# gregbugaj/marie-icr

Measured on AMD Instinct MI355X. Metric: pages/sec (2550x3300, ~40 lines/page), higher is better.
Workload: dtype f16; 1 GPU; BASELINE configs[2]: full detect->crop->recognize, 64 synthetic 2550x3300x3 u8 pages per GPU per step resident in HBM; DiT-base Mask R-CNN detector (resize to 1035x800, 1 pass, 8 pages per forward) + TrOCR-base recognizer on the generator's 40 ground-truth line boxes per page (fixed work), beam 3, 15+1 decoder steps; seeded random weights; f16 operands with fp32 accumulation is the 16-bit mode of ; crops_per_page=40

## Files before the change

### include/marie_hip.h

```cpp
#ifndef MARIE_HIP_H
#define MARIE_HIP_H

#include <stddef.h>
#include <stdint.h>

#ifdef __cplusplus
extern "C" {
#endif

#define MHIP_OK 0
#define MHIP_EINVAL (-22)
#define MHIP_ENOMEM (-12)
#define MHIP_EHIP (-5)
#define MHIP_ESTATE (-1)

#define MHIP_PREC_F16 0
#define MHIP_PREC_F32 1

typedef struct mhip_ctx mhip_ctx;
typedef struct mhip_crnn mhip_crnn;

int mhip_init(int device_id, mhip_ctx** out);
int mhip_destroy(mhip_ctx* ctx);
const char* mhip_last_error(mhip_ctx* ctx);
int mhip_set_stream(mhip_ctx* ctx, void* hip_stream);
int mhip_synchronize(mhip_ctx* ctx);
int mhip_device_info(mhip_ctx* ctx, char* arch, size_t arch_len, int* cu_count, size_t* hbm_bytes);
int mhip_memcpy_dev(mhip_ctx* ctx, void* dst_dev, const void* src_dev, size_t bytes);

typedef struct mhip_gate mhip_gate;
int mhip_gate_create(mhip_ctx* ctx, mhip_gate** out);
int mhip_gate_destroy(mhip_gate* g);
int mhip_gate_signal(mhip_gate* g, mhip_ctx* ctx);
long long mhip_gate_count(mhip_gate* g);
int mhip_gate_open(mhip_gate* g, int open);
int mhip_gate_wait(mhip_gate* g, mhip_ctx* ctx, long long seq, int timeout_ms);

int mhip_profile_enable(mhip_ctx* ctx, int enable);
int mhip_profile_reset(mhip_ctx* ctx);
int mhip_profile_read(mhip_ctx* ctx, int kernel_id, double* total_ms, int64_t* launches);
int mhip_profile_flops(mhip_ctx* ctx, int kernel_id, double* flops);
int mhip_kernel_count(void);
const char* mhip_kernel_name(int kernel_id);

typedef struct mhip_conv_desc {
  int32_t B, H, W, Cin;
  int32_t KH, KW, pad;
  int32_t N;
  int32_t pool, relu, out_f32;
  int32_t dil;
  int32_t Cin1;
  int32_t ldc;
  int32_t pad_cols_writable;
} mhip_conv_desc;
int mhip_conv2d_nhwc(mhip_ctx* ctx, int precision, const mhip_conv_desc* d, const void* in_dev,
                     const void* in2_dev, const void* w_dev, const float* scale_dev, const float* bias_dev,
                     void* out_dev);
typedef struct mhip_conv_ex_desc {
  int32_t B, H, W, Cin;
  int32_t KH, KW, pad;
  int32_t N;
  int32_t pool, relu, out_f32;
  int32_t dil;
  int32_t Cin1;
  int32_t ldc;
  int32_t pad_cols_writable;
  int32_t sy;
  int32_t pad_x;
  int32_t row_period, row_stride, row_offset;
  const void* res_dev;
} mhip_conv_ex_desc;
int mhip_conv2d_nhwc_ex(mhip_ctx* ctx, int precision, const mhip_conv_ex_desc* d, const void* in_dev,
                        const void* in2_dev, const void* w_dev, const float* scale_dev, const float* bias_dev,
                        void* out_dev);

typedef struct mhip_crop_desc {
  uint64_t src_offset;
  int32_t h, w, row_stride, channels;
} mhip_crop_desc;
// ... 359 lines not shown
```

### marie_icr_amd/_lib.py

```python
from __future__ import annotations

import ctypes as C
import os
import weakref

import numpy as np

_HERE = os.path.dirname(os.path.abspath(__file__))
LIB_PATH = os.environ.get("MARIE_HIP_LIB") or os.path.join(_HERE, "libmarie_hip.so")

PREC_F16 = 0
PREC_F32 = 1

_vp, _i, _sz = C.c_void_p, C.c_int, C.c_size_t
_SIGNATURES = (
    ("mhip_init", _i, [_i, C.POINTER(_vp)]),
    ("mhip_destroy", _i, [_vp]),
    ("mhip_last_error", C.c_char_p, [_vp]),
    ("mhip_set_stream", _i, [_vp, _vp]),
    ("mhip_synchronize", _i, [_vp]),
    ("mhip_device_info", _i, [_vp, C.c_char_p, _sz, C.POINTER(_i), C.POINTER(_sz)]),
    ("mhip_memcpy_dev", _i, [_vp, _vp, _vp, _sz]),
    ("mhip_gate_create", _i, [_vp, C.POINTER(_vp)]),
    ("mhip_gate_destroy", _i, [_vp]),
    ("mhip_gate_signal", _i, [_vp, _vp]),
    ("mhip_gate_count", C.c_longlong, [_vp]),
    ("mhip_gate_open", _i, [_vp, _i]),
    ("mhip_gate_wait", _i, [_vp, _vp, C.c_longlong, _i]),
    ("mhip_profile_enable", _i, [_vp, _i]),
    ("mhip_profile_reset", _i, [_vp]),
    ("mhip_profile_read", _i, [_vp, _i, C.POINTER(C.c_double), C.POINTER(C.c_int64)]),
    ("mhip_profile_flops", _i, [_vp, _i, C.POINTER(C.c_double)]),
    ("mhip_kernel_count", _i, []),
    ("mhip_kernel_name", C.c_char_p, [_i]),
    ("mhip_conv2d_nhwc", _i, [_vp, _i, _vp, _vp, _vp, _vp, _vp, _vp, _vp]),
    ("mhip_conv2d_nhwc_ex", _i, [_vp, _i, _vp, _vp, _vp, _vp, _vp, _vp, _vp]),
    ("mhip_icr_create", _i, [_vp, _i, _i, C.POINTER(_vp)]),
    ("mhip_icr_destroy", _i, [_vp]),
    ("mhip_icr_set_tensor", _i, [_vp, C.c_char_p, _vp, C.POINTER(C.c_int64), _i]),
    ("mhip_icr_finalize", _i, [_vp]),
    ("mhip_icr_alloc_arena", _i, [_vp]),
    ("mhip_icr_arena", _i, [_vp, C.POINTER(_vp), C.POINTER(_sz)]),
    ("mhip_icr_steps", _i, []),
    ("mhip_icr_forward", _i, [_vp, _vp, _i, _vp, _vp, _vp, _vp]),
    ("mhip_icr_forward_host", _i, [_vp, _vp, _i, _vp, _vp, _vp, _vp]),
    ("mhip_craft_create", _i, [_vp, _i, C.POINTER(_vp)]),
    ("mhip_craft_destroy", _i, [_vp]),
    ("mhip_craft_set_tensor", _i, [_vp, C.c_char_p, _vp, C.POINTER(C.c_int64), _i]),
    ("mhip_craft_finalize", _i, [_vp]),
    ("mhip_craft_alloc_arena", _i, [_vp]),
    ("mhip_craft_arena", _i, [_vp, C.POINTER(_vp), C.POINTER(_sz)]),
    ("mhip_craft_geometry", _i, [_i, _i, _i, C.c_double, C.POINTER(C.c_double), C.POINTER(_i), C.POINTER(_i),
                                 C.POINTER(_i), C.POINTER(_i)]),
    ("mhip_craft_workspace_bytes", _sz, [_vp, _i, _i, _i, C.c_double]),
    ("mhip_craft_kernel_flops", C.c_double, [_vp, _i, _i, _i, _i, C.c_double]),
    ("mhip_craft_forward", _i, [_vp, _vp, _i, _i, _i, C.c_double, _vp]),
    ("mhip_craft_detect", _i, [_vp, _vp, _i, _i, _i, C.c_double, C.c_float, C.c_float, C.c_float, _vp, _i,
                               C.POINTER(_i), _vp, C.POINTER(C.c_double)]),
    ("mhip_craft_detect_host", _i, [_vp, _vp, _i, _i, _i, C.c_double, C.c_float, C.c_float, C.c_float, _vp, _i,
                                    C.POINTER(_i), _vp, C.POINTER(C.c_double)]),
    ("mhip_craft_boxes_host", _i, [_vp, _vp, _i, _i, C.c_float, C.c_float, C.c_float, _vp, _i, C.POINTER(_i), _vp, _vp,
                                   _vp, _i, C.POINTER(_i)]),
    ("mhip_crop_batch", _i, [_vp, _vp, _vp, _i, _i, _vp]),
    ("mhip_pil_resize_rgb_host", _i, [_vp, _vp, _i, _i, _vp, _i, _i, _i]),
    ("mhip_pil_resize_fragments_host", _i, [_vp, _vp, _sz, _vp, _i, _i, _i, _i, _vp]),
    ("mhip_vit_create", _i, [_vp, _i, _vp, C.POINTER(_vp)]),
    ("mhip_vit_destroy", _i, [_vp]),
    ("mhip_vit_set_tensor", _i, [_vp, C.c_char_p, _vp, C.POINTER(C.c_int64), _i]),
    ("mhip_vit_finalize", _i, [_vp]),
    ("mhip_vit_alloc_arena", _i, [_vp]),
    ("mhip_vit_arena", _i, [_vp, C.POINTER(_vp), C.POINTER(_sz)]),
    ("mhip_vit_forward_host", _i, [_vp, _vp, _i, _i, _i, _i, _i, _i, _vp, _vp, _vp, _vp, _vp]),
    ("mhip_dit_default_config", _i, [_i, _vp]),
# ... 139 lines not shown


class VitConfig(C.Structure):
    _fields_ = [("dim", C.c_int), ("depth", C.c_int), ("heads", C.c_int), ("patch", C.c_int), ("pos_h", C.c_int),
                ("pos_w", C.c_int), ("layer_scale", C.c_int), ("qkv_bias", C.c_int), ("final_norm", C.c_int),
                ("fpn", C.c_int), ("taps", C.c_int * 4), ("ln_eps", C.c_float)]


class DitConfig(C.Structure):
    _fields_ = [("model", C.c_int), ("min_size_test", C.c_int), ("max_size_test", C.c_int),
                ("detections_per_image", C.c_int), ("anchor_sizes", C.c_float * 5), ("aspect_ratios", C.c_float * 3),
                ("rpn_nms_thresh", C.c_float), ("score_thresh", C.c_float), ("nms_thresh", C.c_float),
                ("num_classes", C.c_int)]


class RegisterDesc(C.Structure):
    _fields_ = [("crop_x", C.c_int), ("crop_y", C.c_int), ("crop_w", C.c_int), ("crop_h", C.c_int), ("out_w", C.c_int),
                ("out_h", C.c_int), ("left", C.c_int), ("top", C.c_int), ("canvas_w", C.c_int), ("canvas_h", C.c_int),
                ("n_markers", C.c_int), ("marker_x", C.c_int * 4), ("marker_y", C.c_int * 4), ("marker_radius", C.c_int),
                ("marker_color", C.c_int * 3), ("final_w", C.c_int), ("final_h", C.c_int)]


class TrocrConfig(C.Structure):
    _fields_ = [("enc_dim", C.c_int), ("enc_depth", C.c_int), ("enc_heads", C.c_int), ("dec_dim", C.c_int),
                ("dec_layers", C.c_int), ("dec_heads", C.c_int), ("dec_ffn", C.c_int), ("vocab", C.c_int),
                ("max_positions", C.c_int), ("beam", C.c_int), ("max_len_b", C.c_int), ("min_len", C.c_int),
                ("pad", C.c_int), ("eos", C.c_int), ("embed_scale", C.c_float), ("img_size", C.c_int)]


class LayoutLMv3Config(C.Structure):
    _fields_ = [("hidden", C.c_int), ("layers", C.c_int), ("heads", C.c_int), ("ffn", C.c_int), ("vocab", C.c_int),
                ("type_vocab", C.c_int), ("max_position_embeddings", C.c_int), ("max_2d_position_embeddings", C.c_int),
                ("coordinate_size", C.c_int), ("shape_size", C.c_int), ("input_size", C.c_int), ("patch", C.c_int),
                ("rel_pos_bins", C.c_int), ("max_rel_pos", C.c_int), ("rel_2d_pos_bins", C.c_int),
                ("max_rel_2d_pos", C.c_int), ("layer_norm_eps", C.c_float), ("pad_id", C.c_int), ("num_labels", C.c_int),
                ("max_text", C.c_int)]


class ClipVisConfig(C.Structure):
    _fields_ = [("dim", C.c_int), ("depth", C.c_int), ("heads", C.c_int), ("patch", C.c_int), ("image_size", C.c_int),
                ("ffn", C.c_int), ("proj_dim", C.c_int), ("ln_eps", C.c_float)]


class VqFilters(C.Structure):
    _fields_ = [("n", C.c_int32), ("taps", (C.c_float * 16) * 6), ("dil", (C.c_int32 * 2) * 6), ("weight", C.c_double * 6)]


class CropDesc(C.Structure):
    _fields_ = [("src_offset", C.c_uint64), ("h", C.c_int32), ("w", C.c_int32), ("row_stride", C.c_int32),
                ("channels", C.c_int32)]


POOL_NONE, POOL_2x2, POOL_2x1 = 0, 1, 2

_lib = None


class MarieHipError(RuntimeError):
    pass


def load():
    global _lib
    if _lib is not None:
        return _lib
    import importlib.util
    import sys

    if "torch" not in sys.modules and importlib.util.find_spec("torch") is not None:
        import torch
    if not os.path.exists(LIB_PATH):
        raise MarieHipError(
            f"{LIB_PATH} is missing — the HIP extension is not built; there is no CPU fallback "
            "(run __graft_entry__.build() or `make -C marie_icr_amd/csrc`)")
    lib = C.CDLL(LIB_PATH)
    for name, res, args in _SIGNATURES:
        fn = getattr(lib, name)
        fn.restype = res
        fn.argtypes = args
    _lib = lib
    return lib


def check(ctx_handle, rc: int, what: str):
    if rc != 0:
        msg = load().mhip_last_error(ctx_handle)
        raise MarieHipError(f"{what} failed ({rc}): {msg.decode() if msg else ''}")


class Context:

    def __init__(self, device_id: int = 0):
        lib = load()
        h = C.c_void_p()
        rc = lib.mhip_init(int(device_id), C.byref(h))
        if rc != 0 or not h.value:
            raise MarieHipError(f"mhip_init(device={device_id}) failed ({rc}): no usable HIP device")
        self.h = h
        self.lib = lib
        self.device_id = int(device_id)
        self._children = weakref.WeakSet()

    def adopt(self, child):
        self._children.add(child)

    def set_stream(self, stream_handle: int | None):
        check(self.h, self.lib.mhip_set_stream(self.h, C.c_void_p(stream_handle or 0)), "mhip_set_stream")

    def synchronize(self):
        check(self.h, self.lib.mhip_synchronize(self.h), "mhip_synchronize")

    def device_info(self):
        arch = C.create_string_buffer(64)
        cu = C.c_int()
        hbm = C.c_size_t()
        check(self.h, self.lib.mhip_device_info(self.h, arch, 64, C.byref(cu), C.byref(hbm)), "mhip_device_info")
        return {"arch": arch.value.decode(), "cu_count": cu.value, "hbm_bytes": hbm.value}

    def memcpy_dev(self, dst_ptr: int, src_ptr: int, nbytes: int):
        check(self.h, self.lib.mhip_memcpy_dev(self.h, C.c_void_p(dst_ptr), C.c_void_p(src_ptr), int(nbytes)),
              "mhip_memcpy_dev")

    def conv2d_nhwc(self, precision: int, desc: "ConvDesc", in_ptr: int, w_ptr: int, scale_ptr: int, bias_ptr: int,
                    out_ptr: int, in2_ptr: int = 0):
        check(self.h, self.lib.mhip_conv2d_nhwc(self.h, int(precision), C.byref(desc), C.c_void_p(in_ptr),
                                                C.c_void_p(in2_ptr or 0), C.c_void_p(w_ptr), C.c_void_p(scale_ptr or 0),
                                                C.c_void_p(bias_ptr or 0), C.c_void_p(out_ptr)),
              "mhip_conv2d_nhwc")

    def conv2d_nhwc_ex(self, precision: int, desc: "ConvExDesc", in_ptr: int, w_ptr: int, scale_ptr: int, bias_ptr: int,
                       out_ptr: int, in2_ptr: int = 0):
        check(self.h, self.lib.mhip_conv2d_nhwc_ex(self.h, int(precision), C.byref(desc), C.c_void_p(in_ptr),
                                                   C.c_void_p(in2_ptr or 0), C.c_void_p(w_ptr), C.c_void_p(scale_ptr or 0),
                                                   C.c_void_p(bias_ptr or 0), C.c_void_p(out_ptr)),
              "mhip_conv2d_nhwc_ex")

    def gemm_ln_fold(self, precision: int, desc: "GemmFoldDesc"):
        check(self.h, self.lib.mhip_gemm_ln_fold(self.h, int(precision), C.byref(desc)), "mhip_gemm_ln_fold")

    def ln_finalize(self, stats_ptr: int, chunks: int, ld: int, rstd_ptr: int, mur_ptr: int, rows: int, D: int, eps: float):
        check(self.h, self.lib.mhip_ln_finalize(self.h, C.c_void_p(stats_ptr), int(chunks), int(ld), C.c_void_p(rstd_ptr),
                                                C.c_void_p(mur_ptr), int(rows), int(D), float(eps)), "mhip_ln_finalize")

    def token_init_split(self, hi_ptr: int, lo_ptr: int, cls_row_ptr: int, cls_stats_ptr: int, stats_ptr: int, stats_ld: int,
                         B: int, npad: int, n_tok: int, D: int):
        check(self.h, self.lib.mhip_token_init_split(self.h, C.c_void_p(hi_ptr), C.c_void_p(lo_ptr), C.c_void_p(cls_row_ptr),
                                                     C.c_void_p(cls_stats_ptr), C.c_void_p(stats_ptr), int(stats_ld), int(B),
                                                     int(npad), int(n_tok), int(D)), "mhip_token_init_split")

    def profile_enable(self, on: bool):
        check(self.h, self.lib.mhip_profile_enable(self.h, 1 if on else 0), "mhip_profile_enable")

    def profile_reset(self):
        check(self.h, self.lib.mhip_profile_reset(self.h), "mhip_profile_reset")

    def profile_read(self):
        out = {}
        for k in range(self.lib.mhip_kernel_count()):
            ms = C.c_double()
            n = C.c_int64()
            check(self.h, self.lib.mhip_profile_read(self.h, k, C.byref(ms), C.byref(n)), "mhip_profile_read")
            fl = C.c_double()
            check(self.h, self.lib.mhip_profile_flops(self.h, k, C.byref(fl)), "mhip_profile_flops")
            out[self.lib.mhip_kernel_name(k).decode()] = {"id": k, "total_ms": ms.value, "launches": n.value,
# ... 107 lines not shown
```

### marie_icr_amd/csrc/common.h

```cpp
#pragma once
#include <hip/hip_runtime.h>
#include <stdint.h>
#include <stdio.h>
#include <string.h>

#include <mutex>
#include <string>
#include <vector>

#include "../../include/marie_hip.h"

enum MhipKernelId {
  MHIP_K_CONV_FIRST = 0,
  MHIP_K_CONV_IGEMM = 1,
  MHIP_K_LSTM_REC = 2,
  MHIP_K_CTC_DECODE = 3,
  MHIP_K_IMAGE_OPS = 4,
  MHIP_K_CCL = 5,
  MHIP_K_CROP_BATCH = 6,
  MHIP_K_ATTN = 7,
  MHIP_K_ATTN_FLASH = 8,
  MHIP_K_VIT_OPS = 9,
  MHIP_K_DET_OPS = 10,
  MHIP_K_DEC_OPS = 11,
  MHIP_K_IGEMM_T64 = 12,
  MHIP_K_IGEMM_T128 = 13,
  MHIP_K_IGEMM_T256 = 14,
  MHIP_K_IGEMM_S128 = 15,
  MHIP_K_IGEMM_PATCH = 16,
  MHIP_K_CROSS_ATTN = 17,
  MHIP_K_ATTN_BIAS = 18,
  MHIP_K_VQ_ASSIGN = 19,
  MHIP_K_VQ_KMEANS = 20,
  MHIP_K_VQ_HEATMAP = 21,
  MHIP_K_VQ_PEAKS = 22,
  MHIP_K_CLIP_COSINE = 23,
  MHIP_K_CLIPVIS_PATCHIFY = 24,
  MHIP_K_CLIPVIS_EMBED = 25,
  MHIP_K_QUICK_GELU = 26,
  MHIP_K_CLIPVIS_HEAD = 27,
  MHIP_K_PAIR_COSINE = 28,
  MHIP_K_COUNT = 29
};

constexpr int MHIP_ZERO_BYTES = 65536;

struct ProfSlot {
  double total_ms = 0.0;
  int64_t launches = 0;
  double flops = 0.0;
  int parent = -1;
  std::vector<std::pair<hipEvent_t, hipEvent_t>> pending;
};

struct mhip_ctx {
  int device = 0;
  hipStream_t stream = nullptr;
  std::string err;
  void* ws = nullptr;
  size_t ws_bytes = 0;
  void* zeros = nullptr;
  bool profiling = false;
  ProfSlot prof[MHIP_K_COUNT];
  std::vector<hipEvent_t> event_pool;
  struct PinnedRing {
    static constexpr int N = 4;
    void* buf[N] = {nullptr, nullptr, nullptr, nullptr};
    size_t cap[N] = {0, 0, 0, 0};
    hipEvent_t ev[N] = {nullptr, nullptr, nullptr, nullptr};
    int next = 0;
  } stage;
};
int mhip_stage_h2d(mhip_ctx* ctx, void* dst_dev, const void* src_host, size_t bytes);

int mhip_fail(mhip_ctx* ctx, int code, const char* fmt, ...);
inline void mhip_quiesce(const mhip_ctx* ctx) {
  if (ctx) (void)hipSetDevice(ctx->device);
  (void)hipDeviceSynchronize();
}
int mhip_ensure_workspace(mhip_ctx* ctx, size_t bytes);

struct Carver {
  char* base;
  size_t align;
  size_t off = 0;
  explicit Carver(void* b, size_t a = 256) : base((char*)b), align(a) {}
  template <typename P = char>
  P* take(size_t bytes) {
    const size_t at = off;
    off = (off + bytes + align - 1) / align * align;
    return base ? (P*)(base + at) : nullptr;
  }
  Carver sub(size_t a) const { return Carver(base ? base + off : nullptr, a); }
};

template <typename F>
size_t mhip_layout_bytes(F&& layout, size_t align = 256) {
  Carver c(nullptr, align);
  layout(c);
  return c.off;
}
template <typename F>
int mhip_carve_workspace(mhip_ctx* ctx, F&& layout, size_t align = 256) {
  const size_t need = mhip_layout_bytes(layout, align);
  int rc = mhip_ensure_workspace(ctx, need);
  if (rc) return rc;
  Carver ws(ctx->ws, align);
  layout(ws);
  if (ws.off != need) return mhip_fail(ctx, MHIP_ESTATE, "workspace layout carved %zu bytes, sized %zu", ws.off, need);
  return MHIP_OK;
}
extern "C" int mhip_gate_signal(mhip_gate* g, mhip_ctx* ctx);
void mhip_prof_begin(mhip_ctx* ctx, int kid, hipEvent_t* e0);
void mhip_prof_end(mhip_ctx* ctx, int kid, hipEvent_t e0);

// ... 379 lines not shown
```

### marie_icr_amd/csrc/context.hip

```cpp
#include <stdarg.h>

#include <algorithm>

#include "common.h"

int mhip_fail(mhip_ctx* ctx, int code, const char* fmt, ...) {
  char buf[512];
  va_list ap;
  va_start(ap, fmt);
  vsnprintf(buf, sizeof(buf), fmt, ap);
  va_end(ap);
  if (ctx) ctx->err = buf;
  return code;
}

static const char* kKernelNames[MHIP_K_COUNT] = {"conv_first", "conv_igemm", "lstm_rec",   "ctc_decode",
                                                 "image_ops",  "ccl",        "crop_batch", "attn",
                                                 "attn_flash", "vit_ops",    "det_ops",    "dec_ops",
                                                 "conv_igemm<64>", "conv_igemm<128>", "conv_igemm<256>", "conv_igemm<1128>",
                                                 "conv3x3_patch", "cross_attn", "attn_bias",
                                                 "vq_assign", "vq_kmeans", "vq_heatmap", "vq_peaks", "clip_cosine",
                                                 "clipvis_patchify", "clipvis_embed", "quick_gelu", "clipvis_head", "pair_cosine"};

extern "C" int mhip_kernel_count(void) { return MHIP_K_COUNT; }
extern "C" const char* mhip_kernel_name(int k) { return (k >= 0 && k < MHIP_K_COUNT) ? kKernelNames[k] : ""; }

extern "C" int mhip_init(int device_id, mhip_ctx** out) {
  if (!out) return MHIP_EINVAL;
  *out = nullptr;
  int ndev = 0;
  if (hipGetDeviceCount(&ndev) != hipSuccess || ndev <= 0) return MHIP_EHIP;
  if (device_id < 0 || device_id >= ndev) return MHIP_EINVAL;
  if (hipSetDevice(device_id) != hipSuccess) return MHIP_EHIP;
  mhip_ctx* ctx = new mhip_ctx();
  ctx->device = device_id;
  for (int k = MHIP_K_IGEMM_T64; k <= MHIP_K_IGEMM_PATCH; ++k) ctx->prof[k].parent = MHIP_K_CONV_IGEMM;
  if (hipMalloc(&ctx->zeros, MHIP_ZERO_BYTES) != hipSuccess || hipMemset(ctx->zeros, 0, MHIP_ZERO_BYTES) != hipSuccess) {
    delete ctx;
    return MHIP_ENOMEM;
  }
  *out = ctx;
  return MHIP_OK;
}

extern "C" int mhip_destroy(mhip_ctx* ctx) {
  if (!ctx) return MHIP_OK;
  (void)hipSetDevice(ctx->device);
  mhip_quiesce(ctx);
  for (auto& s : ctx->prof)
    for (auto& p : s.pending) {
      (void)hipEventDestroy(p.first);
      (void)hipEventDestroy(p.second);
    }
  for (auto e : ctx->event_pool) (void)hipEventDestroy(e);
  for (int i = 0; i < mhip_ctx::PinnedRing::N; ++i) {
    if (ctx->stage.ev[i]) (void)hipEventDestroy(ctx->stage.ev[i]);
    if (ctx->stage.buf[i]) (void)hipHostFree(ctx->stage.buf[i]);
  }
  if (ctx->ws) (void)hipFree(ctx->ws);
  if (ctx->zeros) (void)hipFree(ctx->zeros);
  delete ctx;
  return MHIP_OK;
}

int mhip_stage_h2d(mhip_ctx* ctx, void* dst_dev, const void* src_host, size_t bytes) {
  if (!bytes) return MHIP_OK;
  mhip_ctx::PinnedRing& r = ctx->stage;
  const int i = r.next;
  r.next = (i + 1) % mhip_ctx::PinnedRing::N;
  if (r.ev[i]) MHIP_HIP(ctx, hipEventSynchronize(r.ev[i]));
  else MHIP_HIP(ctx, hipEventCreateWithFlags(&r.ev[i], hipEventDisableTiming));
  if (bytes > r.cap[i]) {
    if (r.buf[i]) (void)hipHostFree(r.buf[i]);
    r.buf[i] = nullptr; r.cap[i] = 0;
    const size_t cap = std::max<size_t>(bytes, 64 * 1024);
    MHIP_HIP(ctx, hipHostMalloc(&r.buf[i], cap, hipHostMallocDefault));
    r.cap[i] = cap;
  }
  memcpy(r.buf[i], src_host, bytes);
  MHIP_HIP(ctx, hipMemcpyAsync(dst_dev, r.buf[i], bytes, hipMemcpyHostToDevice, ctx->stream));
  MHIP_HIP(ctx, hipEventRecord(r.ev[i], ctx->stream));
  return MHIP_OK;
}

extern "C" const char* mhip_last_error(mhip_ctx* ctx) { return ctx ? ctx->err.c_str() : "null ctx"; }

extern "C" int mhip_set_stream(mhip_ctx* ctx, void* s) {
  if (!ctx) return MHIP_EINVAL;
  ctx->stream = (hipStream_t)s;
  return MHIP_OK;
}

extern "C" int mhip_synchronize(mhip_ctx* ctx) {
  if (!ctx) return MHIP_EINVAL;
  MHIP_HIP(ctx, hipStreamSynchronize(ctx->stream));
  return MHIP_OK;
}

extern "C" int mhip_device_info(mhip_ctx* ctx, char* arch, size_t arch_len, int* cu_count, size_t* hbm_bytes) {
  if (!ctx) return MHIP_EINVAL;
  hipDeviceProp_t p;
  MHIP_HIP(ctx, hipGetDeviceProperties(&p, ctx->device));
  if (arch && arch_len) {
    strncpy(arch, p.gcnArchName, arch_len - 1);
    arch[arch_len - 1] = 0;
  }
  if (cu_count) *cu_count = p.multiProcessorCount;
  if (hbm_bytes) *hbm_bytes = p.totalGlobalMem;
  return MHIP_OK;
}

extern "C" int mhip_memcpy_dev(mhip_ctx* ctx, void* dst, const void* src, size_t bytes) {
  if (!ctx || (bytes && (!dst || !src))) return MHIP_EINVAL;
  MHIP_HIP(ctx, hipMemcpyAsync(dst, src, bytes, hipMemcpyDeviceToDevice, ctx->stream));
  return MHIP_OK;
}

int mhip_ensure_workspace(mhip_ctx* ctx, size_t bytes) {
  if (bytes <= ctx->ws_bytes) return MHIP_OK;
  MHIP_HIP(ctx, hipStreamSynchronize(ctx->stream));
  if (ctx->ws) MHIP_HIP(ctx, hipFree(ctx->ws));
  ctx->ws = nullptr;
  ctx->ws_bytes = 0;
  size_t want = bytes + bytes / 8;
  if (hipMalloc(&ctx->ws, want) != hipSuccess) {
    (void)hipGetLastError();
    return mhip_fail(ctx, MHIP_ENOMEM, "workspace allocation of %zu bytes failed", want);
  }
  ctx->ws_bytes = want;
  return MHIP_OK;
}

static hipEvent_t get_event(mhip_ctx* ctx) {
  if (!ctx->event_pool.empty()) {
    hipEvent_t e = ctx->event_pool.back();
    ctx->event_pool.pop_back();
    return e;
  }
  hipEvent_t e = nullptr;
  (void)hipEventCreate(&e);
  return e;
}
// ... 58 lines not shown
```

### marie_icr_amd/csrc/conv_igemm.hip

```cpp
#include <stdlib.h>

#include <type_traits>

#include "igemm_common.h"

using namespace igemm;

namespace {

template <int BN_>
struct Cfg {
  static constexpr bool SMALL = BN_ / 1000 == 1;
  static constexpr int BN = BN_ % 1000;
  static constexpr int BM = SMALL ? 128 : ((BN == 64) ? 512 : 256);
  static constexpr int WN = BN / 64;
  static constexpr int WM = 8 / WN;
  static constexpr int MT = BM / WM / 16;
  static constexpr int NSTAGE = SMALL ? 4 : ((BN == 128) ? 3 : 2);
  static constexpr int A_BYTES = BM * ROWB;
  static constexpr int B_BYTES = BN * ROWB;
  static constexpr int STAGE_BYTES = A_BYTES + B_BYTES;
  static constexpr int RPI = 64 * 16 / ROWB;
  static constexpr int ACHUNKS = BM * (ROWB / 16) / NTHREADS;
  static constexpr int WCHUNKS = BN * (ROWB / 16) / NTHREADS;
  static constexpr int GL = ACHUNKS + WCHUNKS;
  static constexpr int EPW = BN < 128 ? BN : 128;
  static constexpr int EPI_BYTES = BM * (EPW * 4 + 16);
  static constexpr int RING_BYTES = NSTAGE * STAGE_BYTES;
  static constexpr int LDS_BYTES = RING_BYTES > EPI_BYTES ? RING_BYTES : EPI_BYTES;
};

__device__ __forceinline__ float gelu_erf(float t) {
  const float x = t * 0.70710678118654752f, ax = fabsf(x);
  const float u = __builtin_amdgcn_rcpf(__builtin_fmaf(0.3275911f, ax, 1.f));
  float poly = __builtin_fmaf(1.061405429f, u, -1.453152027f);
  poly = __builtin_fmaf(poly, u, 1.421413741f);
  poly = __builtin_fmaf(poly, u, -0.284496736f);
  poly = __builtin_fmaf(poly, u, 0.254829592f);
  poly = poly * u;
  const float e = __builtin_fmaf(-poly, __builtin_amdgcn_exp2f((-1.4426950408889634f * ax) * ax), 1.f);
  const float h = 0.5f * t;
  return __builtin_fmaf(h, copysignf(e, x), h);
}

template <int CTRL>
__device__ __forceinline__ float dpp_f(float v) {
  return __builtin_bit_cast(float, __builtin_amdgcn_update_dpp(0, __builtin_bit_cast(int, v), CTRL, 0xf, 0xf, true));
}
__device__ __forceinline__ float sum8(float v) {
  v += dpp_f<0xB1>(v);
  v += dpp_f<0x4E>(v);
  v += dpp_f<0x141>(v);
  return v;
}


__device__ __forceinline__ void staged8(const char* src, float (&f)[8]) {
  const float4v a0 = *(const float4v*)src, a1 = *(const float4v*)(src + 16);
  f[0] = a0[0]; f[1] = a0[1]; f[2] = a0[2]; f[3] = a0[3]; f[4] = a1[0]; f[5] = a1[1]; f[6] = a1[2]; f[7] = a1[3];
}


template <bool SMALL, typename V, typename P>
__device__ __forceinline__ void tile_store(const V& v, P dst) {
  if (SMALL) *dst = v;
  else __builtin_nontemporal_store(v, dst);
}

template <int POOL>
__device__ __forceinline__ void decode_row(const IgemmArgs& p, int m, int& b, int& y, int& x) {
  if (POOL == POOL_NONE) {
    x = m % p.Wo;
    int r = m / p.Wo;
    y = r % p.Ho;
    b = r / p.Ho;
  } else if (POOL == POOL_2x2) {
    int sub = m & 3, q = m >> 2;
    int xp = q % p.Wp;
    int r = q / p.Wp;
    int yp = r % p.Hp;
    b = r / p.Hp;
    y = 2 * yp + (sub >> 1);
    x = 2 * xp + (sub & 1);
  } else {
    int sub = m & 1, q = m >> 1;
    x = q % p.Wo;
    int r = q / p.Wo;
    int yp = r % p.Hp;
    b = r / p.Hp;
    y = 2 * yp + sub;
  }
}

template <typename T, int POOL, int BN_, bool DUAL, int EPI = EPI_NONE>
__global__ __launch_bounds__(NTHREADS) void conv_igemm_kernel(IgemmArgs p) {
  extern __shared__ __attribute__((aligned(16))) char smem[];
  typedef Cfg<BN_> C;
  typedef typename Tr<T>::chunk_t chunk_t;
  constexpr int E = Tr<T>::E;
  constexpr int BKE = ROWB / sizeof(T);
  constexpr int MT = C::MT;
  constexpr int WROWS = MT * 16;
  constexpr int BM = C::BM;
  constexpr int A_BYTES = C::A_BYTES;

  const int tid = threadIdx.x, lane = tid & 63, wave = tid >> 6;

  int mt, nt;
  {
    const int nblk = gridDim.x, bid = blockIdx.x;
    const int q = nblk >> 3, r = nblk & 7, xcd = bid & 7;
    const int L = (xcd < r ? xcd * (q + 1) : r * (q + 1) + (xcd - r) * q) + (bid >> 3);
    nt = L % p.ntiles;
    mt = L / p.ntiles;
  }
  const int m0 = mt * BM, n0 = nt * C::BN;

  constexpr int RPI = C::RPI, RSTEP = RPI * 8;
  const int srow = wave * RPI + (lane >> 3);
  const int lchunk = (lane & 7) ^ ((srow >> 1) & 7);
  const char* a_src[C::ACHUNKS];
  int a_y[C::ACHUNKS], a_x[C::ACHUNKS];
  const char* w_src[C::WCHUNKS];
  const bool pure = !DUAL && POOL == POOL_NONE && p.KH == 1 && p.KW == 1 && p.pad == 0 && p.pad_x == 0 &&
                    p.sy == 1 && (size_t)p.Ktot * sizeof(T) + ROWB <= (size_t)MHIP_ZERO_BYTES;
#pragma unroll
  for (int q = 0; q < C::ACHUNKS; ++q) {
    int m = m0 + q * RSTEP + srow;
    if (pure) {
      a_y[q] = a_x[q] = 0;
      a_src[q] = p.in + ((size_t)m * p.Cin + (size_t)lchunk * E) * sizeof(T);
      continue;
    }
    int b = 0, y = -100000, x = -100000;
    if (m < p.M) decode_row<POOL>(p, m, b, y, x);
    a_y[q] = y;
    a_x[q] = x;
    if (m < p.M) {
      y = y * p.sy - p.pad;
      x = x - p.pad_x;
      a_y[q] = y;
      a_x[q] = x;
    }
    size_t pix = ((size_t)b * p.H + y) * p.W + x;
    if (DUAL) a_src[q] = (const char*)pix;
    else a_src[q] = p.in + (pix * p.Cin + (size_t)lchunk * E) * sizeof(T);
  }
#pragma unroll
  for (int q = 0; q < C::WCHUNKS; ++q) {
    int n = n0 + q * RSTEP + srow;
    w_src[q] = (n < p.N) ? p.w + ((size_t)n * p.Ktot + (size_t)lchunk * E) * sizeof(T) : nullptr;
  }

  const int wave_s = __builtin_amdgcn_readfirstlane(wave);
  if (pure) {
#pragma unroll
    for (int q = 0; q < C::ACHUNKS; ++q)
      if (m0 + q * RSTEP + srow >= p.M) a_src[q] = p.zeros + lchunk * 16;
#pragma unroll
    for (int q = 0; q < C::WCHUNKS; ++q)
      if (!w_src[q]) w_src[q] = p.zeros + lchunk * 16;
  }
  auto stage_pure = [&](int slot) {
    char* la = smem + slot * C::STAGE_BYTES + wave_s * RPI * ROWB;
    char* lb = la + A_BYTES;
#pragma unroll
    for (int q = 0; q < C::ACHUNKS; ++q) {
// ... 629 lines not shown
  a.Wo = d.W + 2 * a.pad_x - a.dil * (d.KW - 1);
  if (a.res && d.pool != POOL_NONE) return mhip_fail(ctx, MHIP_EINVAL, "conv_igemm: a residual needs an unpooled output");
  if (a.res && d.relu == ACT_GELU) return mhip_fail(ctx, MHIP_EINVAL, "conv_igemm: GELU is applied before any residual add");
  if (a.ldc && (a.ldc < d.N || d.pool != POOL_NONE))
    return mhip_fail(ctx, MHIP_EINVAL, "conv_igemm: bad output pitch %d", a.ldc);
  if ((a.res || a.ldc) && ((size_t)(a.ldc ? a.ldc : d.N) * (d.out_f32 ? 4 : esz)) % 16 != 0)
    return mhip_fail(ctx, MHIP_EINVAL, "conv_igemm: residual / pitched outputs need 16-byte aligned rows");
  a.epi = d.epi;
  a.ln_a = d.ln_a; a.ln_b = d.ln_b; a.ln_cs = d.ln_cs; a.row_bias = d.row_bias;
  a.out2 = (char*)d.out2; a.res2 = (const char*)d.res2; a.stats = d.stats; a.stats_ld = d.stats_ld;
  if (d.epi != EPI_NONE) {
    const long long Mrows = (long long)d.B * d.H * d.W;
    if (precision != MHIP_PREC_F16 || d.KH != 1 || d.KW != 1 || d.pad != 0 || d.pool != POOL_NONE || d.in2 || d.out_f32 || d.ldc ||
        d.N % 8 != 0 || (d.epi != EPI_SPLIT && Mrows % 4 != 0) || (d.sy > 1))
      return mhip_fail(ctx, MHIP_EINVAL, "conv_igemm: a LayerNorm-folded epilogue needs a plain f16 GEMM (N %% 8 == 0, M %% 4 == 0)");
    if (d.epi == EPI_SPLIT && (!d.out2 || !d.res || !d.res2 || !d.stats || d.stats_ld <= 0 || d.N % 64 != 0 || d.relu != ACT_NONE))
      return mhip_fail(ctx, MHIP_EINVAL, "conv_igemm: the split epilogue needs both planes of output and residual, a statistics buffer and N %% 64 == 0");
    if (d.epi == EPI_LN_ROWS && (!d.ln_a || !d.ln_b || !d.ln_cs || d.res || d.row_period)) return mhip_fail(ctx, MHIP_EINVAL, "conv_igemm: EPI_LN_ROWS operands");
    if (d.epi == EPI_LN_COLS && (!d.ln_a || !d.ln_b || !d.ln_cs || !d.row_bias || d.res || d.relu != ACT_NONE || d.row_period))
      return mhip_fail(ctx, MHIP_EINVAL, "conv_igemm: EPI_LN_COLS operands");
    if (((unsigned long long)d.out | (unsigned long long)d.out2 | (unsigned long long)d.res | (unsigned long long)d.res2 |
         (unsigned long long)d.ln_a | (unsigned long long)d.ln_b | (unsigned long long)d.ln_cs | (unsigned long long)d.row_bias) & 15)
      return mhip_fail(ctx, MHIP_EINVAL, "conv_igemm: LayerNorm-folded epilogue operands must be 16-byte aligned");
  }
  a.in2 = (const char*)d.in2;
  a.Cin1 = d.in2 ? d.Cin1 : d.Cin;
  if (d.in2) {
    if (d.KH != 1 || d.KW != 1 || d.pad != 0 || d.pool != POOL_NONE)
      return mhip_fail(ctx, MHIP_EINVAL, "conv_igemm: a concatenated input needs a 1x1, unpadded, unpooled conv");
    if (d.Cin1 <= 0 || d.Cin1 >= d.Cin || d.Cin1 % bke != 0)
      return mhip_fail(ctx, MHIP_EINVAL, "conv_igemm: Cin1=%d must split Cin=%d on a multiple of %d", d.Cin1, d.Cin, bke);
  }
  if (a.Ho <= 0 || a.Wo <= 0) return mhip_fail(ctx, MHIP_EINVAL, "conv_igemm: empty output %dx%d", a.Ho, a.Wo);
  a.Hp = a.Ho; a.Wp = a.Wo;
  long long M;
  if (d.pool == POOL_2x2) {
    a.Hp = a.Ho / 2; a.Wp = a.Wo / 2;
    M = (long long)d.B * a.Hp * a.Wp * 4;
  } else if (d.pool == POOL_2x1) {
    a.Hp = a.Ho / 2;
    M = (long long)d.B * a.Hp * a.Wo * 2;
  } else {
    M = (long long)d.B * a.Ho * a.Wo;
  }
  if (M <= 0 || M > 0x7fffffffLL - 512) return mhip_fail(ctx, MHIP_EINVAL, "conv_igemm: M=%lld out of range", M);
  a.M = (int)M;
  a.N = d.N;
  a.Ktot = d.KH * d.KW * d.Cin;
  a.cpt = d.Cin / bke;
  a.nslices = d.KH * d.KW * a.cpt;
  a.relu = d.relu;
  a.out_f32 = d.out_f32;
  a.PH = a.PW = a.tiles_x = a.tiles_y = 0;
  const double fl = ctx->profiling ? mhip_conv_flops(d) : 0.0;
  if (ctx->profiling) ctx->prof[MHIP_K_CONV_IGEMM].flops += fl;
  if (d.epi == EPI_NONE) {
    const int r = mhip_try_launch_conv3x3_patch(ctx, precision, d, a);
    if (r == 0) ctx->prof[MHIP_K_IGEMM_PATCH].flops += fl;
    if (r <= 0) return r;
  }
  static const int force_bn = getenv("MARIE_HIP_FORCE_BN") ? atoi(getenv("MARIE_HIP_FORCE_BN")) : 0;
  const int bn = force_bn ? force_bn : ((a.N > 128) ? 256 : ((a.N > 64 || d.epi != EPI_NONE) ? 128 : 64));
  const int bm = (bn == 64) ? 512 : 256;
  a.mtiles = (a.M + bm - 1) / bm;
  a.ntiles = (a.N + bn - 1) / bn;
  static const bool mid_off = getenv("MARIE_HIP_NO_MID_TILE") != nullptr;
  int tile = bn == 256 ? 256 : (bn == 128 ? 128 : 64);
  if (!mid_off && bn == 256 && a.mtiles * a.ntiles < 192 && a.mtiles * ((a.N + 127) / 128) >= 192 && !force_bn) {
    a.ntiles = (a.N + 127) / 128;
    ctx->prof[MHIP_K_IGEMM_T128].flops += fl;
    tile = 128;
  } else if (a.mtiles * a.ntiles < 192 && (a.N > 64 || d.epi != EPI_NONE) && d.pool == POOL_NONE && !d.in2) {
    a.mtiles = (a.M + 127) / 128;
    a.ntiles = (a.N + 127) / 128;
    ctx->prof[MHIP_K_IGEMM_S128].flops += fl;
    tile = 1128;
  } else {
    ctx->prof[bn == 64 ? MHIP_K_IGEMM_T64 : (bn == 128 ? MHIP_K_IGEMM_T128 : MHIP_K_IGEMM_T256)].flops += fl;
  }
  return precision == MHIP_PREC_F16 ? launch_tile<_Float16>(ctx, a, d.pool, tile) : launch_tile<float>(ctx, a, d.pool, tile);
}
```

### marie_icr_amd/csrc/igemm_common.h

```cpp
#pragma once
#include "common.h"

typedef _Float16 half8 __attribute__((ext_vector_type(8)));
typedef float float4v __attribute__((ext_vector_type(4)));
typedef unsigned int uint4v __attribute__((ext_vector_type(4)));

namespace igemm {

constexpr int ROWB = 128;
constexpr int NTHREADS = 512;

struct IgemmArgs {
  const char* in;
  const char* w;
  const float* scale;
  const float* bias;
  char* out;
  const char* zeros;
  int B, H, W, Cin;
  int KH, KW, pad;
  int Ho, Wo, Hp, Wp;
  int N, M;
  int Ktot;
  int nslices;
  int cpt;
  int relu, out_f32;
  int mtiles, ntiles;
  int dil;
  const char* in2;
  int Cin1;
  int sy;
  int pad_x;
  const char* res;
  int ldc;
  int pad_ok;
  int row_period;
  int row_stride;
  int row_offset;
  int PH, PW;
  int tiles_x, tiles_y;
  int epi;
  const float* ln_a;
  const float* ln_b;
  const float* ln_cs;
  const float* row_bias;
  char* out2;
  const char* res2;
  float* stats;
  int stats_ld;
};

template <typename T>
struct Tr;
template <>
struct Tr<_Float16> {
  static constexpr int E = 8;
  typedef half8 chunk_t;
  static __device__ __forceinline__ void mma(const chunk_t& a, const chunk_t& b, float4v& c) {
    c = __builtin_amdgcn_mfma_f32_16x16x32_f16(a, b, c, 0, 0, 0);
  }
};
template <>
struct Tr<float> {
  static constexpr int E = 4;
  typedef float4v chunk_t;
  static __device__ __forceinline__ void mma(const chunk_t& a, const chunk_t& b, float4v& c) {
    c = __builtin_amdgcn_mfma_f32_16x16x4f32(a[0], b[0], c, 0, 0, 0);
    c = __builtin_amdgcn_mfma_f32_16x16x4f32(a[1], b[1], c, 0, 0, 0);
    c = __builtin_amdgcn_mfma_f32_16x16x4f32(a[2], b[2], c, 0, 0, 0);
    c = __builtin_amdgcn_mfma_f32_16x16x4f32(a[3], b[3], c, 0, 0, 0);
  }
};

__device__ __forceinline__ void glds16(const void* gsrc, void* lds_wave_base) {
  __builtin_amdgcn_global_load_lds((const __attribute__((address_space(1))) void*)gsrc,
                                   (__attribute__((address_space(3))) void*)lds_wave_base, 16, 0, 0);
}


template <typename OT>
__device__ __forceinline__ void lds_put(char* base, int pitch, int row, int col, float v) {
  *(OT*)(base + row * pitch + col * (int)sizeof(OT)) = (OT)v;
}

}

int mhip_try_launch_conv3x3_patch(mhip_ctx* ctx, int precision, const ConvDesc& d, igemm::IgemmArgs& a);
```

Before: 95.52 pages/s.

## Add L2-aware grouped tile walk planner for 1x1 conv GEMMs

Replaces the fixed row-major tile ordering of the implicit-GEMM conv kernel with a configurable banded walk (group N-tiles or M-tiles), chosen by a host-side L2 traffic model for plain 1x1 GEMMs. The aim is to cut redundant HBM/L2 refetches of activation and weight tiles across XCDs. The planner only switches away from the legacy order when its modelled traffic falls below half of the baseline, so many shapes keep the old order. It also adds an API and an environment variable to force or disable the walk.

```diff
diff --git a/include/marie_hip.h b/include/marie_hip.h
--- a/include/marie_hip.h
+++ b/include/marie_hip.h
@@ -25,6 +25,9 @@
 const char* mhip_last_error(mhip_ctx* ctx);
 int mhip_set_stream(mhip_ctx* ctx, void* hip_stream);
 int mhip_synchronize(mhip_ctx* ctx);
+enum { MHIP_WALK_PLANNER = 0, MHIP_WALK_LEGACY = 1, MHIP_WALK_FORCED = 2 };
+enum { MHIP_WALK_FAMILY_N = 0, MHIP_WALK_FAMILY_M = 1 };
+int mhip_set_tile_walk(mhip_ctx* ctx, int mode, int family, int group);
 int mhip_device_info(mhip_ctx* ctx, char* arch, size_t arch_len, int* cu_count, size_t* hbm_bytes);
 int mhip_memcpy_dev(mhip_ctx* ctx, void* dst_dev, const void* src_dev, size_t bytes);
 
diff --git a/marie_icr_amd/_lib.py b/marie_icr_amd/_lib.py
--- a/marie_icr_amd/_lib.py
+++ b/marie_icr_amd/_lib.py
@@ -19,6 +19,7 @@
     ("mhip_last_error", C.c_char_p, [_vp]),
     ("mhip_set_stream", _i, [_vp, _vp]),
     ("mhip_synchronize", _i, [_vp]),
+    ("mhip_set_tile_walk", _i, [_vp, _i, _i, _i]),
     ("mhip_device_info", _i, [_vp, C.c_char_p, _sz, C.POINTER(_i), C.POINTER(_sz)]),
     ("mhip_memcpy_dev", _i, [_vp, _vp, _vp, _sz]),
     ("mhip_gate_create", _i, [_vp, C.POINTER(_vp)]),
@@ -264,6 +265,8 @@
 
 
 POOL_NONE, POOL_2x2, POOL_2x1 = 0, 1, 2
+WALK_MODES = {"planner": 0, "legacy": 1, "forced": 2}
+WALK_FAMILIES = {"N": 0, "M": 1}
 
 _lib = None
 
@@ -322,6 +325,10 @@
     def synchronize(self):
         check(self.h, self.lib.mhip_synchronize(self.h), "mhip_synchronize")
 
+    def set_tile_walk(self, mode: str = "planner", family: str = "N", group: int = 0):
+        check(self.h, self.lib.mhip_set_tile_walk(self.h, WALK_MODES[mode], WALK_FAMILIES[family], int(group)),
+              "mhip_set_tile_walk")
+
     def device_info(self):
         arch = C.create_string_buffer(64)
         cu = C.c_int()
diff --git a/marie_icr_amd/csrc/common.h b/marie_icr_amd/csrc/common.h
--- a/marie_icr_amd/csrc/common.h
+++ b/marie_icr_amd/csrc/common.h
@@ -61,6 +61,8 @@
   size_t ws_bytes = 0;
   void* zeros = nullptr;
   bool profiling = false;
+  int walk_mode = 0, walk_family = 0, walk_group = 0;
+  int walk_last_family = 0, walk_last_group = 0;
   ProfSlot prof[MHIP_K_COUNT];
   std::vector<hipEvent_t> event_pool;
   struct PinnedRing {
diff --git a/marie_icr_amd/csrc/context.hip b/marie_icr_amd/csrc/context.hip
--- a/marie_icr_amd/csrc/context.hip
+++ b/marie_icr_amd/csrc/context.hip
@@ -1,8 +1,10 @@
 #include <stdarg.h>
+#include <stdlib.h>
 
 #include <algorithm>
 
 #include "common.h"
+#include "tile_walk.h"
 
 int mhip_fail(mhip_ctx* ctx, int code, const char* fmt, ...) {
   char buf[512];
@@ -34,6 +36,8 @@
   if (hipSetDevice(device_id) != hipSuccess) return MHIP_EHIP;
   mhip_ctx* ctx = new mhip_ctx();
   ctx->device = device_id;
+  const char* walk = getenv("MARIE_HIP_TILE_WALK");
+  if (walk && !strcmp(walk, "legacy")) ctx->walk_mode = tile_walk::MODE_LEGACY;
   for (int k = MHIP_K_IGEMM_T64; k <= MHIP_K_IGEMM_PATCH; ++k) ctx->prof[k].parent = MHIP_K_CONV_IGEMM;
   if (hipMalloc(&ctx->zeros, MHIP_ZERO_BYTES) != hipSuccess || hipMemset(ctx->zeros, 0, MHIP_ZERO_BYTES) != hipSuccess) {
     delete ctx;
@@ -88,6 +92,21 @@
 extern "C" int mhip_set_stream(mhip_ctx* ctx, void* s) {
   if (!ctx) return MHIP_EINVAL;
   ctx->stream = (hipStream_t)s;
+  return MHIP_OK;
+}
+
+extern "C" int mhip_set_tile_walk(mhip_ctx* ctx, int mode, int family, int group) {
+  if (!ctx) return MHIP_EINVAL;
+  if (mode != MHIP_WALK_PLANNER && mode != MHIP_WALK_LEGACY && mode != MHIP_WALK_FORCED)
+    return mhip_fail(ctx, MHIP_EINVAL, "mhip_set_tile_walk: unknown mode %d", mode);
+  if (mode == MHIP_WALK_FORCED && ((family != MHIP_WALK_FAMILY_N && family != MHIP_WALK_FAMILY_M) || group < 1))
+    return mhip_fail(ctx, MHIP_EINVAL, "mhip_set_tile_walk: family %d, group %d", family, group);
+  static_assert(MHIP_WALK_PLANNER == tile_walk::MODE_PLANNER && MHIP_WALK_LEGACY == tile_walk::MODE_LEGACY &&
+                MHIP_WALK_FORCED == tile_walk::MODE_FORCED && MHIP_WALK_FAMILY_N == tile_walk::FAMILY_N &&
+                MHIP_WALK_FAMILY_M == tile_walk::FAMILY_M, "include/marie_hip.h and tile_walk.h agree");
+  ctx->walk_mode = mode;
+  ctx->walk_family = mode == MHIP_WALK_FORCED ? family : 0;
+  ctx->walk_group = mode == MHIP_WALK_FORCED ? group : 0;
   return MHIP_OK;
 }
 
diff --git a/marie_icr_amd/csrc/conv_igemm.hip b/marie_icr_amd/csrc/conv_igemm.hip
--- a/marie_icr_amd/csrc/conv_igemm.hip
+++ b/marie_icr_amd/csrc/conv_igemm.hip
@@ -3,6 +3,7 @@
 #include <type_traits>
 
 #include "igemm_common.h"
+#include "tile_walk.h"
 
 using namespace igemm;
 
@@ -108,11 +109,8 @@
 
   int mt, nt;
   {
-    const int nblk = gridDim.x, bid = blockIdx.x;
-    const int q = nblk >> 3, r = nblk & 7, xcd = bid & 7;
-    const int L = (xcd < r ? xcd * (q + 1) : r * (q + 1) + (xcd - r) * q) + (bid >> 3);
-    nt = L % p.ntiles;
-    mt = L / p.ntiles;
+    const int L = tile_walk::xcd_linear_index(blockIdx.x, gridDim.x);
+    tile_walk::walk_tile(L, p.mtiles, p.ntiles, p.walk_family, p.walk_group, mt, nt);
   }
   const int m0 = mt * BM, n0 = nt * C::BN;
 
@@ -848,6 +846,7 @@
   a.relu = d.relu;
   a.out_f32 = d.out_f32;
   a.PH = a.PW = a.tiles_x = a.tiles_y = 0;
+  a.walk_family = tile_walk::FAMILY_N; a.walk_group = 0;
   const double fl = ctx->profiling ? mhip_conv_flops(d) : 0.0;
   if (ctx->profiling) ctx->prof[MHIP_K_CONV_IGEMM].flops += fl;
   if (d.epi == EPI_NONE) {
@@ -874,5 +873,17 @@
   } else {
     ctx->prof[bn == 64 ? MHIP_K_IGEMM_T64 : (bn == 128 ? MHIP_K_IGEMM_T128 : MHIP_K_IGEMM_T256)].flops += fl;
   }
+  a.walk_family = tile_walk::FAMILY_N;
+  a.walk_group = a.ntiles;
+  const bool plain_gemm = d.KH == 1 && d.KW == 1 && a.pad == 0 && a.pad_x == 0 && a.sy == 1 && d.pool == POOL_NONE && !d.in2;
+  if (plain_gemm && ctx->walk_mode != tile_walk::MODE_LEGACY) {
+    const int tbn = tile == 1128 ? 128 : tile, tbm = tile == 1128 ? 128 : (tile == 64 ? 512 : 256);
+    const tile_walk::Walk w = ctx->walk_mode == tile_walk::MODE_FORCED ? tile_walk::Walk{ctx->walk_family, ctx->walk_group}
+                                                                       : tile_walk::plan_tile_walk(a.mtiles, a.ntiles, tbm, tbn, a.Ktot, esz);
+    a.walk_family = w.family;
+    a.walk_group = w.group;
+  }
+  ctx->walk_last_family = a.walk_family;
+  ctx->walk_last_group = a.walk_group;
   return precision == MHIP_PREC_F16 ? launch_tile<_Float16>(ctx, a, d.pool, tile) : launch_tile<float>(ctx, a, d.pool, tile);
 }
diff --git a/marie_icr_amd/csrc/igemm_common.h b/marie_icr_amd/csrc/igemm_common.h
--- a/marie_icr_amd/csrc/igemm_common.h
+++ b/marie_icr_amd/csrc/igemm_common.h
@@ -48,6 +48,8 @@
   const char* res2;
   float* stats;
   int stats_ld;
+  alignas(8) int walk_family;
+  int walk_group;
 };
 
 template <typename T>
diff --git a/marie_icr_amd/csrc/tile_walk.h b/marie_icr_amd/csrc/tile_walk.h
--- /dev/null
+++ b/marie_icr_amd/csrc/tile_walk.h
@@ -0,0 +1,91 @@
+#pragma once
+
+#if defined(__HIPCC__)
+#define TW_HD __host__ __device__
+#else
+#define TW_HD
+#endif
+
+namespace tile_walk {
+
+enum { FAMILY_N = 0, FAMILY_M = 1 };
+enum { MODE_PLANNER = 0, MODE_LEGACY = 1, MODE_FORCED = 2 };
+
+constexpr int XCDS = 8;
+constexpr int TILES_IN_FLIGHT = 32;
+constexpr long long L2_BYTES = 4ll << 20;
+
+TW_HD inline int xcd_linear_index(int bid, int nblk) {
+  const int q = nblk >> 3, r = nblk & 7, xcd = bid & 7;
+  return (xcd < r ? xcd * (q + 1) : r * (q + 1) + (xcd - r) * q) + (bid >> 3);
+}
+
+TW_HD inline void walk_tile(int L, int mtiles, int ntiles, int family, int group, int& mt, int& nt) {
+  const int banded = family == FAMILY_M ? mtiles : ntiles;
+  const int slow = family == FAMILY_M ? ntiles : mtiles;
+  const int g = group < 1 ? 1 : (group > banded ? banded : group);
+  const int per_band = slow * g;
+  const int band = L / per_band;
+  const int rem = L - band * per_band;
+  const int f0 = band * g;
+  const int w = banded - f0 < g ? banded - f0 : g;
+  const int s = rem / w;
+  const int f = f0 + (rem - s * w);
+  mt = family == FAMILY_M ? f : s;
+  nt = family == FAMILY_M ? s : f;
+}
+
+struct Walk {
+  int family, group;
+};
+
+inline double walk_cost(int mtiles, int ntiles, double tA, double tW, int family, int group) {
+  const int banded = family == FAMILY_M ? mtiles : ntiles, slow = family == FAMILY_M ? ntiles : mtiles;
+  const double tF = family == FAMILY_M ? tA : tW, tS = family == FAMILY_M ? tW : tA;
+  const int g = group < 1 ? 1 : (group > banded ? banded : group);
+  double total = 0;
+  for (int f0 = 0; f0 < banded; f0 += g) {
+    const int w = banded - f0 < g ? banded - f0 : g;
+    double b = w < TILES_IN_FLIGHT ? w : TILES_IN_FLIGHT, a = TILES_IN_FLIGHT / b;
+    if (a > slow) {
+      a = slow;
+      b = (double)TILES_IN_FLIGHT / slow;
+      if (b > banded) b = banded;
+    }
+    const double resident = (w > b ? w : b) * tF;
+    if (resident + a * tS <= (double)L2_BYTES) {
+      double xcds = (double)XCDS * w / banded + (g < banded ? 1.0 : 0.0);
+      if (xcds > XCDS) xcds = XCDS;
+      total += slow * tS + xcds * w * tF;
+    } else {
+      const double rounds = (double)slow * w / TILES_IN_FLIGHT;
+      total += rounds * (a * tS + b * tF);
+    }
+  }
+  return total;
+}
+
+constexpr double MIN_MODELLED_RATIO = 0.5;
+
+inline Walk plan_tile_walk(int mtiles, int ntiles, int BM, int BN, int Ktot, int esz) {
+  const Walk legacy = {FAMILY_N, ntiles};
+  if (mtiles < 1 || ntiles < 1) return legacy;
+  const double tA = (double)BM * Ktot * esz, tW = (double)BN * Ktot * esz;
+  const double base = walk_cost(mtiles, ntiles, tA, tW, FAMILY_N, ntiles);
+  static const int groups[] = {1, 2, 3, 4, 6, 8, 12, 16};
+  Walk best = legacy;
+  double best_cost = base;
+  for (int family = FAMILY_N; family <= FAMILY_M; ++family) {
+    const int banded = family == FAMILY_M ? mtiles : ntiles;
+    for (int k = 0; k <= 8; ++k) {
+      const int g = k < 8 ? groups[k] : banded;
+      if (k < 8 && g >= banded) continue;
+      if (family == FAMILY_N && g == ntiles) continue;
+      const double c = walk_cost(mtiles, ntiles, tA, tW, family, g);
+      if (c < best_cost) { best = Walk{family, g}; best_cost = c; }
+    }
+  }
+  return best_cost < MIN_MODELLED_RATIO * base ? best : legacy;
+}
+
+}
```

Result: no change. 96.02 pages/s, median of 6 (+0.5%).
